# abdenlab/giql

Measured on AMD Instinct MI355X. Metric: overlap-pairs/sec, 10Mx100M INTERSECTS inner join, higher is better.
Workload: dtype int32

## Files before the change

giql_amd/csrc/giql_hip.hip:

```cpp
#include <hip/hip_runtime.h>
#include <chrono>
#include <atomic>
#include <sys/mman.h>
#include <utility>
#if defined(__SSE2__)
#include <emmintrin.h>
#endif
#include <mutex>
#include <thread>
#include <stdarg.h>
#include <stdio.h>
#include <stdlib.h>
#include <string.h>

#include <vector>

#include "../../include/giql_hip.h"
#include "aux_kernels.hip.h"
#include "take_kernels.hip.h"
#include "select_kernels.hip.h"
#include "cluster_kernels.hip.h"
#include "dev_common.hip.h"
#include "join_kernels.hip.h"
#include "onesweep.hip.h"
// ... 24 lines not shown

#define GIQL_TRY(expr)      \
  do {                      \
    int _rc = (expr);       \
    if (_rc != GIQL_OK) return _rc; \
  } while (0)

#ifndef GIQL_RC_ITEMS
#define GIQL_RC_ITEMS 1
#endif
constexpr int RC_ITEMS_C2 = GIQL_RC_ITEMS;
#ifndef GIQL_FILL_ITEMS
#define GIQL_FILL_ITEMS 16
#endif
constexpr int FILL_ITEMS_C2 = GIQL_FILL_ITEMS;

#ifndef GIQL_STREAM_GRID
#define GIQL_STREAM_GRID 16384u
#endif

static inline size_t align_up(size_t x, size_t a) { return (x + a - 1) / a * a; }
static inline u32 cdiv(u64 a, u64 b) { return (u32)((a + b - 1) / b); }

struct SortBufs {
  u32* key[2];
  u32* end[2];
  u32* rid[2];
};

struct InnerState {
  SortBufs sa, sb;
  u32 nt1 = 0, nt2 = 0;
  int c1_items = C1_ITEMS_MAX;
  u32* wlo1 = nullptr;
  u64* c1_base = nullptr;
  bool c1_fill = false;
  u32 *lo1 = nullptr, *cnt1 = nullptr;
  u64* off1 = nullptr;
  u32* wlo2 = nullptr;
  u32* lo2 = nullptr;
  u32* cnt2 = nullptr;
  u64* off2 = nullptr;
  int uniform = 0;
};

constexpr size_t C1_SMALL_ROWS = (size_t)4 << 20;
constexpr u64 OVERLAP_MAX_ROWS = (u64)4 << 20;

struct Switches {
  bool classic_sort = false;
  int os_variant = 0;
  int os_order = 2;
  u32 os_help_after = OS_HELP_AFTER;
  int inject_timeout = 0;
  bool no_uniform = false;
  bool no_span_hist = false;
  bool no_coarse_b = false;
  double coarse_max_group_rows = 8.0;
  bool no_fuse_count = false;
  bool no_local_sort = false;
  u64 local_min_rows = 1u << 21;
  double local_min_bucket_rows = 300.0;
  double local_max_bucket_rows = 2800.0;
  bool no_narrow = false;
  int force_bits = 0;
};

struct Guesses {
  bool local_sort = true;
  int os_order = 2;
  int inject_timeout = 0;
  u64 last_span = 0;
  bool last_no_irr = false;
  bool nearest_two_sorts = false;
  int nearest_aligned = -1;
  bool spec_valid = false;
  int spec_form = 0;
  i64 spec_len = 0;
  bool spec_aligned = false;
  bool spec_fuse_len_ok = false;
  bool spec_sorted[2] = {false, false};
  bool row_spec_valid = false;
  i64 row_spec_len = 0;
  int spec_misses = 0;
  int local_resorts = 0;
  int order_fallbacks = 0;
};

struct CallState {
  bool prezeroed = false;
  bool first_unstable = false;
  u32* span_hist_dirty[2] = {nullptr, nullptr};
  int force_local = 0;
  int index_bits = 16;
  bool used_sorted[2] = {false, false};
  bool last_sort_local = false;
  int last_local_bits = 16;
  bool count_fused = false;
  bool bucket_join = false;
};

struct InnerPlan {
  bool planned = false;
  bool plan_is_join = false;
  bool swapped = false;
  int32_t* fuse_a = nullptr;
// ... 331 lines not shown
    if (offs[k] > omax) omax = offs[k];
  }
  hipLaunchKernelGGL(k_chrom_offsets, dim3(1), dim3(256), 0, st, lb.gmin, lb.gmax, n_chrom, omin,
                     omax, lb.chrom_base, lb.chrom_first, ctx->d_meta, lb.len_part, nblk[0], nblk[1],
                     hist ? 1 : 0, lb.abase);
  return post_launch("spans");
}

static int run_linearize(giql_hip_ctx* ctx, hipStream_t st, const giql_side& s, int n_chrom,
                         const LinBufs& lb, u32* keys, u32* ends, u32* irr_list, int which,
                         int keep_irregular, u32* hist_partial = nullptr, u32* gbase = nullptr,
                         u32* hist_end = nullptr, u32* gbase_end = nullptr, bool skip_end = false) {
  if (s.n == 0) return GIQL_OK;
  const int* end_col = skip_end ? (const int*)nullptr : s.end;
  bool dirty = false;
  for (int k = 0; k < 2; k++)
    if (hist_partial && ctx->call.span_hist_dirty[k] == hist_partial) {
      dirty = true;
      ctx->call.span_hist_dirty[k] = nullptr;
    }
  if (hist_partial && (!ctx->call.prezeroed || dirty))
    HIP_TRY(hipMemsetAsync(hist_partial, 0, (size_t)LIN_HIST_REPLICAS * 1024 * sizeof(u32), st));
  if (hist_end && !ctx->call.prezeroed)
    HIP_TRY(hipMemsetAsync(hist_end, 0, (size_t)LIN_HIST_REPLICAS * 1024 * sizeof(u32), st));
  Phase ph(ctx, st, GIQL_PH_LINEARIZE, hist_partial ? 2 : 1);
  u32 grid = cdiv((u64)s.n, LIN_NT);
  if (grid > (u32)LIN_MAX_BLOCKS) grid = LIN_MAX_BLOCKS;
  if (hist_end)
    hipLaunchKernelGGL((k_linearize<true>), dim3(grid), dim3(LIN_NT), 0, st, s.chrom, s.start, end_col,
                       (u32)s.n, s.start_off, s.end_off, n_chrom, lb.chrom_base, keys, ends, irr_list,
                       ctx->d_meta, which, keep_irregular, hist_partial, hist_end);
  else
    hipLaunchKernelGGL((k_linearize<false>), dim3(grid), dim3(LIN_NT), 0, st, s.chrom, s.start, end_col,
                       (u32)s.n, s.start_off, s.end_off, n_chrom, lb.chrom_base, keys, ends, irr_list,
                       ctx->d_meta, which, keep_irregular, hist_partial, (u32*)nullptr);
  if (hist_partial)
    hipLaunchKernelGGL(k_digit_offsets, dim3(4), dim3(256), 0, st, hist_partial,
                       (u32)LIN_HIST_REPLICAS, gbase);
  if (hist_end)
    hipLaunchKernelGGL(k_digit_offsets, dim3(4), dim3(256), 0, st, hist_end, (u32)LIN_HIST_REPLICAS,
                       gbase_end);
  return post_launch("linearize");
}

static inline size_t os_pass_words(size_t n) {
  return (size_t)cdiv(n ? n : 1, OS_MIN_TILE) * OS_BINS + 16;
}
static inline size_t os_pass_stride(const giql_hip_ctx* ctx, size_t n) {
  return ctx->sw.os_variant == 0 ? (size_t)cdiv(n ? n : 1, 8192) * OS_BINS + 16 : os_pass_words(n);
}

template <int NT, int ITEMS>
static void launch_onesweep(giql_hip_ctx* ctx, hipStream_t st, SortBufs& sb, int src, int dst, bool first,
                            u32 n, int shift, const u32* gbase, u32* status, DevMeta* meta, int unstable = 0) {
  const u32 grid = cdiv(n, NT * ITEMS);
  u32* claim = status + os_pass_stride(ctx, n) - 16;
  const u32* rin = (first || !sb.rid[0]) ? (const u32*)nullptr : sb.rid[src];
  const int mode = (sb.rid[0] ? 1 : 0) | (sb.end[0] ? 2 : 0);
#define GIQL_OS_LAUNCH(M)                                                                            \
  hipLaunchKernelGGL((k_onesweep<M, NT, ITEMS>), dim3(grid), dim3(NT), 0, st, sb.key[src],           \
                     sb.end[0] ? sb.end[src] : (const u32*)nullptr, rin, sb.key[dst],                 \
                     sb.end[0] ? sb.end[dst] : (u32*)nullptr, sb.rid[0] ? sb.rid[dst] : (u32*)nullptr, \
                     n, shift, gbase, status, claim, meta, ctx->guess.os_order, ctx->sw.os_help_after, (const u32*)nullptr, 0u, 0u,  \
                     unstable)
  switch (mode) {
    case 0: GIQL_OS_LAUNCH(0); break;
    case 1: GIQL_OS_LAUNCH(1); break;
    case 2: GIQL_OS_LAUNCH(2); break;
    default: GIQL_OS_LAUNCH(3); break;
  }
#undef GIQL_OS_LAUNCH
}

static inline int density_bits(const giql_hip_ctx* ctx, double per_bucket) {
  int w = 16;
  while (per_bucket > ctx->sw.local_max_bucket_rows && w > BS_MIN_WBITS && !ctx->sw.no_narrow) {
    per_bucket *= 0.5;
    w--;
  }
  return per_bucket <= ctx->sw.local_max_bucket_rows ? w : 0;
}

static inline int sort_local_bits(const giql_hip_ctx* ctx, size_t n) {
  if (ctx->call.force_local > 0 && ctx->bucket_bnd && ctx->sw.os_variant == 0) return ctx->call.index_bits;
  if (ctx->call.force_local < 0) return 0;
  if (!(ctx->guess.local_sort && ctx->bucket_bnd && ctx->sw.os_variant == 0 && n >= ctx->sw.local_min_rows)) return 0;
  const double span = ctx->guess.last_span ? (double)ctx->guess.last_span : 3.2e9;
  double per_bucket = (double)n * 65536.0 / span;
  if (per_bucket < ctx->sw.local_min_bucket_rows) return 0;
  if (ctx->sw.force_bits) return ctx->sw.force_bits;
  return density_bits(ctx, per_bucket);
}
static inline int local_passes(int wbits) { return wbits == 16 ? 2 : 3; }

struct FuseCount {
  BsFuse dev;
  u32 nq_total;
  const u32* irr_q;
  const u32* gbq3;
  u32 key_mask;
  const int* len_max_q;
  u32* zero_ptr;
  u32 zero_words;
  bool join = false;
  bool general = false;
  const int* len_max_u = nullptr;
};

static int64_t bucket_stage_fused_bytes(u32 n, const FuseCount& fuse);
static void launch_bucket_stage_fused(giql_hip_ctx* ctx, hipStream_t st, SortBufs& sb, u32 n, const u32* gbase,
                                      const FuseCount& fuse_in, int wbits = 16) {
  FuseCount fuse = fuse_in;
  fuse.dev.wbits = (u32)wbits;
  const u32 BS_BUCKETS = bs_n_buckets((u32)wbits);
  ctx->stats.phase_bytes[GIQL_PH_SORT_LOCAL] += bucket_stage_fused_bytes(n, fuse);
  ctx->call.count_fused = true;
  ctx->call.bucket_join = fuse.join;
  ctx->call.last_local_bits = wbits;
  {
    Phase ph(ctx, st, GIQL_PH_COUNT, 1);
    hipLaunchKernelGGL(k_bucket_bounds_fused, dim3(cdiv((u64)3 * BS_BUCKETS + 1, 256)), dim3(256), 0, st, sb.key[0], n,
                       gbase + 3 * OS_BINS, ctx->bucket_bnd, ctx->bucket_big, fuse.dev, fuse.nq_total, fuse.irr_q,
                       fuse.gbq3, fuse.key_mask, fuse.len_max_q, fuse.zero_ptr, fuse.zero_words, fuse.len_max_u);
// ... 43 lines not shown
                             int skip_digits = 0, const FuseCount* fuse = nullptr, bool presorted = false) {
  if (n == 0) return GIQL_OK;
  if (presorted) {
    const int mode = (sb.rid[0] ? 1 : 0) | (sb.end[0] ? 2 : 0);
    const int wbits_pre = sort_local_bits(ctx, n);
    const bool local_fused = fuse && mode == (fuse->general ? 3 : 1) && wbits_pre != 0;
    {
      Phase ph(ctx, st, GIQL_PH_SORT_SCATTER, 1);
      u32 grid = cdiv(n, 256 * 8);
      if (grid > GIQL_STREAM_GRID) grid = GIQL_STREAM_GRID;
      if (keygen) {
        ctx->stats.phase_bytes[GIQL_PH_SORT_SCATTER] += (int64_t)4 * n * ((mode & 2 ? 3 : 2) + 1 + (mode & 1) + (mode & 2 ? 1 : 0));
        const u32 so = (u32)keygen->start_off, eo = (u32)keygen->end_off;
        switch (mode) {
          case 0: hipLaunchKernelGGL(k_keygen_stream<0>, dim3(grid), dim3(256), 0, st, keygen->chrom, keygen->start, keygen->end, n, abase, so, eo, sb.key[0], (u32*)nullptr, (u32*)nullptr); break;
          case 1: hipLaunchKernelGGL(k_keygen_stream<1>, dim3(grid), dim3(256), 0, st, keygen->chrom, keygen->start, keygen->end, n, abase, so, eo, sb.key[0], (u32*)nullptr, sb.rid[0]); break;
          case 2: hipLaunchKernelGGL(k_keygen_stream<2>, dim3(grid), dim3(256), 0, st, keygen->chrom, keygen->start, keygen->end, n, abase, so, eo, sb.key[0], sb.end[0], (u32*)nullptr); break;
          default: hipLaunchKernelGGL(k_keygen_stream<3>, dim3(grid), dim3(256), 0, st, keygen->chrom, keygen->start, keygen->end, n, abase, so, eo, sb.key[0], sb.end[0], sb.rid[0]); break;
        }
      } else if (sb.rid[0] && !keep_rids) {
        ctx->stats.phase_bytes[GIQL_PH_SORT_SCATTER] += (int64_t)4 * n;
        hipLaunchKernelGGL(k_iota, dim3(grid), dim3(256), 0, st, sb.rid[0], n);
      }
      GIQL_TRY(post_launch("sorted input (no sort)"));
    }
    if (!local_fused) return GIQL_OK;
    ctx->call.last_sort_local = true;
    launch_bucket_stage_fused(ctx, st, sb, n, gbase, *fuse, wbits_pre);
    return post_launch("bucket stage (sorted input, fused count)");
  }
  const int wbits = sort_local_bits(ctx, n);
  const bool local = wbits != 0;
  if (local) ctx->call.last_sort_local = true;
  if (local) skip_digits = 0;
  const int n_pass = local ? local_passes(wbits) : 4 - skip_digits;
  const int first_digit = local ? 4 - n_pass : skip_digits;
  const size_t per_pass = os_pass_stride(ctx, n);
  if (!ctx->call.prezeroed) HIP_TRY(hipMemsetAsync(status, 0, n_pass * per_pass * sizeof(u32), st));
  {
    Phase ph(ctx, st, GIQL_PH_SORT_SCATTER, n_pass);
    for (int pass = 0; pass < n_pass; pass++) {
      const int src = pass & 1, dst = src ^ 1;
      const int digit = first_digit + pass;
      u32* stat = status + pass * per_pass;
      const bool first = pass == 0 && !keep_rids;
      const u32* gb = gbase + digit * OS_BINS;
      {
        const int w_out = 1 + (sb.rid[0] ? 1 : 0) + (sb.end[0] ? 1 : 0);
        const int w_in = (pass == 0 && keygen) ? 2 + (sb.end[0] ? 1 : 0)
                                               : 1 + ((sb.rid[0] && !first) ? 1 : 0) + (sb.end[0] ? 1 : 0);
        ctx->stats.phase_bytes[GIQL_PH_SORT_SCATTER] += (int64_t)4 * (w_in + w_out) * n;
      }
      const int unstable = (pass == 0 && !keep_rids && ctx->call.first_unstable) ? 1 : 0;
      if (pass == 0 && keygen) {
        const u32 grid = cdiv(n, 1024 * 8);
        u32* claim = stat + per_pass - 16;
        if (sb.end[0])
          hipLaunchKernelGGL((k_onesweep<3, 1024, 8, true>), dim3(grid), dim3(1024), 0, st,
                             reinterpret_cast<const u32*>(keygen->start), reinterpret_cast<const u32*>(keygen->end),
                             reinterpret_cast<const u32*>(keygen->chrom), sb.key[dst], sb.end[dst], sb.rid[dst], n,
                             digit * 8, gb, stat, claim, ctx->d_meta, ctx->guess.os_order, ctx->sw.os_help_after, abase,
                             (u32)keygen->start_off, (u32)keygen->end_off, unstable);
        else
          hipLaunchKernelGGL((k_onesweep<1, 1024, 8, true>), dim3(grid), dim3(1024), 0, st,
                             reinterpret_cast<const u32*>(keygen->start), reinterpret_cast<const u32*>(keygen->chrom),
                             (const u32*)nullptr, sb.key[dst], (u32*)nullptr, sb.rid[dst], n, digit * 8, gb, stat, claim,
                             ctx->d_meta, ctx->guess.os_order, ctx->sw.os_help_after, abase, (u32)keygen->start_off, 0u, unstable);
        continue;
      }
      switch (ctx->sw.os_variant) {
        case 1: launch_onesweep<512, 8>(ctx, st, sb, src, dst, first, n, digit * 8, gb, stat, ctx->d_meta, unstable); break;
        case 2: launch_onesweep<512, 16>(ctx, st, sb, src, dst, first, n, digit * 8, gb, stat, ctx->d_meta, unstable); break;
        case 3: launch_onesweep<256, 16>(ctx, st, sb, src, dst, first, n, digit * 8, gb, stat, ctx->d_meta, unstable); break;
        case 4: launch_onesweep<1024, 4>(ctx, st, sb, src, dst, first, n, digit * 8, gb, stat, ctx->d_meta, unstable); break;
        case 5: case 7: launch_onesweep<1024, 12>(ctx, st, sb, src, dst, first, n, digit * 8, gb, stat, ctx->d_meta, unstable); break;
        default: launch_onesweep<1024, 8>(ctx, st, sb, src, dst, first, n, digit * 8, gb, stat, ctx->d_meta, unstable); break;
      }
    }
  }
  if (n_pass & 1) {
    u32* t;
    t = sb.key[0], sb.key[0] = sb.key[1], sb.key[1] = t;
    t = sb.end[0], sb.end[0] = sb.end[1], sb.end[1] = t;
    t = sb.rid[0], sb.rid[0] = sb.rid[1], sb.rid[1] = t;
  }
  if (local) {
    const int mode = (sb.rid[0] ? 1 : 0) | (sb.end[0] ? 2 : 0);
    if (fuse && mode == (fuse->general ? 3 : 1)) {
      launch_bucket_stage_fused(ctx, st, sb, n, gbase, *fuse, wbits);
      return post_launch("onesweep sort (fused count)");
    }
    BsFuse bw;
    bw.wbits = (u32)wbits;
    ctx->call.last_local_bits = wbits;
    const u32 BS_BUCKETS = bs_n_buckets((u32)wbits);
    HIP_TRY(hipMemsetAsync(ctx->bucket_big, 0, sizeof(u32), st));
    Phase ph(ctx, st, GIQL_PH_SORT_LOCAL, 3);
    ctx->stats.phase_bytes[GIQL_PH_SORT_LOCAL] +=
        (int64_t)8 * (1 + (sb.rid[0] ? 1 : 0) + (sb.end[0] ? 1 : 0)) * n;
    hipLaunchKernelGGL(k_bucket_bounds, dim3(cdiv((u64)BS_BUCKETS + 1, 256)), dim3(256), 0, st, sb.key[0], n,
                       gbase + 3 * OS_BINS, ctx->bucket_bnd, (u32)wbits);
#define GIQL_BS_LAUNCH(M)                                                                              \
  if (wbits == 16)                                                                                     \
    hipLaunchKernelGGL((k_bucket_sort<M, 0, true>), dim3(BS_BUCKETS), dim3(BS_NT), 0, st, sb.key[0],   \
                       sb.end[0] ? sb.end[0] : (u32*)nullptr, sb.rid[0] ? sb.rid[0] : (u32*)nullptr,    \
                       ctx->bucket_bnd, ctx->d_meta, ctx->bucket_big, bw);                             \
  else                                                                                                 \
  hipLaunchKernelGGL((k_bucket_sort<M>), dim3(BS_BUCKETS), dim3(BS_NT), 0, st, sb.key[0],              \
                     sb.end[0] ? sb.end[0] : (u32*)nullptr, sb.rid[0] ? sb.rid[0] : (u32*)nullptr,      \
                     ctx->bucket_bnd, ctx->d_meta, ctx->bucket_big, bw);                               \
  hipLaunchKernelGGL((k_bucket_sort_big<M>), dim3(ctx->n_cu), dim3(BS_NT), 0, st, sb.key[0],           \
                     sb.end[0] ? sb.end[0] : (u32*)nullptr, sb.rid[0] ? sb.rid[0] : (u32*)nullptr,      \
                     sb.key[1], sb.end[0] ? sb.end[1] : (u32*)nullptr, sb.rid[0] ? sb.rid[1] : (u32*)nullptr, \
                     ctx->bucket_bnd, ctx->bucket_big, bw)
    switch (mode) {
      case 0: GIQL_BS_LAUNCH(0); break;
      case 1: GIQL_BS_LAUNCH(1); break;
      case 2: GIQL_BS_LAUNCH(2); break;
      default: GIQL_BS_LAUNCH(3); break;
    }
#undef GIQL_BS_LAUNCH
  }
  return post_launch("onesweep sort");
}

static inline void adopt_by_end(SortBufs& owner, const SortBufs& by_end) {
  for (int k = 0; k < 2; k++) {
    owner.end[k] = by_end.key[k];
    owner.key[k] = by_end.end[k];
// ... 151 lines not shown
  speculated = false;
  if (ctx->sw.no_uniform) return GIQL_OK;
  if (ctx->guess.row_spec_valid) {
    uni_len = ctx->guess.row_spec_len;
    speculated = true;
    return GIQL_OK;
  }
  GIQL_TRY(read_meta(ctx, st));
  uni_len = uniform_len_b(*ctx->h_meta);
  ctx->guess.last_span = ctx->h_meta->total_span;
  return GIQL_OK;
}

static bool row_form_settled(giql_hip_ctx* ctx, i64 uni_len, bool speculated) {
  if (ctx->sw.no_uniform) return true;
  const i64 actual = uniform_len_b(*ctx->h_meta);
  const bool ok = !(speculated && uni_len != 0 && actual != uni_len);
  ctx->guess.row_spec_valid = ok;
  ctx->guess.row_spec_len = actual;
  return ok;
}

static void parse_flag(const char* v, void* f) { *(bool*)f = atoi(v) != 0; }
static void parse_int(const char* v, void* f) { *(int*)f = atoi(v); }
static void parse_u32(const char* v, void* f) { *(u32*)f = (u32)strtoul(v, nullptr, 10); }
static void parse_classic(const char* v, void* f) { *(bool*)f = strcmp(v, "classic") == 0; }
static void parse_positive(const char* v, void* f) {
  if (atof(v) > 0) *(double*)f = atof(v);
}
static void parse_nonnegative(const char* v, void* f) {
  if (atof(v) >= 0) *(double*)f = atof(v);
}
static void parse_local_bits(const char* v, void* f) {
  if (atoi(v) >= BS_MIN_WBITS && atoi(v) <= 16) *(int*)f = atoi(v);
}
static void parse_local_min_rows(const char* v, void* f) {
  Switches& s = *(Switches*)f;
  s.local_min_rows = strtoull(v, nullptr, 10);
  s.local_max_bucket_rows = 1e30;
  s.local_min_bucket_rows = 0.0;
}

static Switches read_switches() {
  Switches s;
  const struct {
    const char* name;
    void (*parse)(const char*, void*);
    void* field;
  } table[] = {
      {"GIQL_HIP_SORT", parse_classic, &s.classic_sort},
      {"GIQL_HIP_OS_VARIANT", parse_int, &s.os_variant},
      {"GIQL_HIP_OS_ORDER", parse_int, &s.os_order},
      {"GIQL_HIP_OS_HELP_AFTER", parse_u32, &s.os_help_after},
      {"GIQL_HIP_INJECT_TIMEOUT", parse_int, &s.inject_timeout},
      {"GIQL_HIP_NO_UNIFORM", parse_flag, &s.no_uniform},
      {"GIQL_HIP_NO_SPAN_HIST", parse_flag, &s.no_span_hist},
      {"GIQL_HIP_NO_COARSE_B", parse_flag, &s.no_coarse_b},
      {"GIQL_HIP_COARSE_MAX_GROUP_ROWS", parse_positive, &s.coarse_max_group_rows},
      {"GIQL_HIP_NO_FUSE_COUNT", parse_flag, &s.no_fuse_count},
      {"GIQL_HIP_NO_LOCAL_SORT", parse_flag, &s.no_local_sort},
      {"GIQL_HIP_LOCAL_MIN_ROWS", parse_local_min_rows, &s},
      {"GIQL_HIP_LOCAL_MIN_BUCKET_ROWS", parse_nonnegative, &s.local_min_bucket_rows},
      {"GIQL_HIP_LOCAL_MAX_BUCKET_ROWS", parse_positive, &s.local_max_bucket_rows},
      {"GIQL_HIP_NO_NARROW_BUCKETS", parse_flag, &s.no_narrow},
      {"GIQL_HIP_LOCAL_BITS", parse_local_bits, &s.force_bits},
  };
  for (const auto& row : table)
    if (const char* v = getenv(row.name)) row.parse(v, row.field);
  return s;
}

extern "C" {

int giql_hip_abi_version(void) { return GIQL_HIP_ABI_VERSION; }

const char* giql_hip_last_error(void) { return g_err; }

int giql_hip_device_count(int* n_devices) {
  if (!n_devices) return set_err(GIQL_ERR_INVALID, "n_devices is NULL");
  int n = 0;
  HIP_TRY(hipGetDeviceCount(&n));
  *n_devices = n;
  return GIQL_OK;
}

int giql_hip_create(int device, giql_hip_ctx** out) {
  if (!out) return set_err(GIQL_ERR_INVALID, "out is NULL");
  *out = nullptr;
  int n = 0;
  HIP_TRY(hipGetDeviceCount(&n));
  if (device < 0 || device >= n)
    return set_err(GIQL_ERR_INVALID, "device %d not in [0,%d)", device, n);
  HIP_TRY(hipSetDevice(device));
  giql_hip_ctx* ctx = new (std::nothrow) giql_hip_ctx(read_switches());
  if (!ctx) return set_err(GIQL_ERR_NOMEM, "out of host memory");
  ctx->device = device;
  memset(&ctx->stats, 0, sizeof(ctx->stats));
  {
    hipDeviceProp_t prop;
    if (hipGetDeviceProperties(&prop, device) == hipSuccess && prop.multiProcessorCount > 0)
      ctx->n_cu = prop.multiProcessorCount;
  }
  hipError_t e = hipMalloc((void**)&ctx->d_meta, sizeof(DevMeta));
  if (e == hipSuccess) e = hipHostMalloc((void**)&ctx->h_meta, sizeof(DevMeta), hipHostMallocDefault);
  if (e == hipSuccess) e = hipMalloc((void**)&ctx->d_scratch64, 64);
  if (e == hipSuccess &&
// ... 2954 lines not shown
```

giql_amd/csrc/onesweep.hip.h:

```cpp
#pragma once

#include "dev_common.hip.h"

namespace giql {

constexpr int OS_BINS = 256;
constexpr int OS_MIN_TILE = 4096;
constexpr u32 OS_FLAG_AGG = 1u << 30;
constexpr u32 OS_FLAG_PREFIX = 2u << 30;
constexpr u32 OS_VALUE_MASK = (1u << 30) - 1u;
constexpr u32 OS_MAX_ROWS = (1u << 30) - 1u;
constexpr u32 OS_NO_TILE = 0xFFFFFFFFu;
#ifndef GIQL_OS_LB_WIDTH
#define GIQL_OS_LB_WIDTH 8
#endif
constexpr int OS_LB_WIDTH = GIQL_OS_LB_WIDTH;
#ifndef GIQL_OS_PRESTAGE
#define GIQL_OS_PRESTAGE 1
#endif

constexpr u32 OS_HELP_AFTER = 1u << 11;

#if defined(GIQL_OS_TIMELINE)
constexpr u32 OS_TL_TILES = 1u << 15;
__device__ unsigned long long g_os_tl[OS_TL_TILES * 16];
#define GIQL_TL(tile, k)                                                             \
  do {                                                                               \
    if (threadIdx.x == 0 && (tile) < OS_TL_TILES) g_os_tl[(size_t)(tile) * 16 + (k)] = wall_clock64(); \
  } while (0)
#else
#define GIQL_TL(tile, k) do { } while (0)
#endif

__device__ __forceinline__ void wave_match8(u32 d, u64 active, u32& below, u32& total) {
  u32 mis_lo = 0, mis_hi = 0;
#pragma unroll
  for (int b = 0; b < 8; b++) {
    const int s = __builtin_amdgcn_sbfe((int)d, b, 1);
    const u64 m = __ballot(s != 0);
    mis_lo |= (u32)m ^ (u32)s;
    mis_hi |= (u32)(m >> 32) ^ (u32)s;
  }
  const u32 p_lo = (u32)active & ~mis_lo;
  const u32 p_hi = (u32)(active >> 32) & ~mis_hi;
  below = __builtin_amdgcn_mbcnt_hi(p_hi, __builtin_amdgcn_mbcnt_lo(p_lo, 0u));
  total = (u32)__popc(p_lo) + (u32)__popc(p_hi);
}

#ifndef GIQL_OS_XCD_GROUP
#define GIQL_OS_XCD_GROUP 16
#endif
constexpr u32 OS_GROUPS = XCD_GROUPS;
constexpr u32 OS_GROUP = GIQL_OS_XCD_GROUP;

__device__ __forceinline__ u32 os_tile_of_ticket(u32 t, u32 n_tiles) { return xcd_tile_of_block<OS_GROUP>(t, n_tiles); }

__device__ __forceinline__ void os_store(u32* p, u32 v) { *p = v; }

template <int PAYLOAD, int OS_NT, int OS_ITEMS, bool FULL, bool KEYGEN = false>
__device__ __forceinline__ u32 onesweep_tile(
    const u32* __restrict__ keys_in, const u32* __restrict__ ends_in, const u32* __restrict__ rids_in,
    u32* __restrict__ keys_out, u32* __restrict__ ends_out, u32* __restrict__ rids_out, u32 n_valid,
    u32 tile, u32 tile_base, int shift, const u32* __restrict__ gbase, u32* __restrict__ status,
    DevMeta* __restrict__ meta, u32* s_buf, u32 (*s_wcnt)[OS_BINS], u32* s_dstart, u32* s_goff,
    u32* s_scan, u32* s_help, u32 help_after, u32 n_total, const u32* s_abase = nullptr, u32 start_off = 0,
    u32 end_off = 0, const bool unstable = false) {
  constexpr int OS_NW = OS_NT / WAVE;
  const u32 tid = threadIdx.x;
  const u32 lane = lane_id();
  const u32 w = wave_id();

  u32 key[OS_ITEMS];
  const u32 wbase = w * (OS_ITEMS * WAVE);
  const u32* kin = keys_in + tile_base;
  const u32* ein = (PAYLOAD & 2) ? ends_in + tile_base : nullptr;
  const u32* rin = ((PAYLOAD & 1) && rids_in && !KEYGEN) ? rids_in + tile_base : nullptr;
  const int* cin = KEYGEN ? reinterpret_cast<const int*>((PAYLOAD & 2) ? rids_in : ends_in) + tile_base : nullptr;
  if (KEYGEN) {
    u32 cc[OS_ITEMS];
#pragma unroll
    for (int i = 0; i < OS_ITEMS; i++) {
      const u32 r = wbase + i * WAVE + lane;
      const bool ok = FULL || r < n_valid;
      cc[i] = ok ? (u32)cin[r] : 0u;
      key[i] = ok ? kin[r] : 0u;
    }
    __syncthreads();
#pragma unroll
    for (int i = 0; i < OS_ITEMS; i++) {
      const u32 r = wbase + i * WAVE + lane;
      const bool ok = FULL || r < n_valid;
      key[i] = ok ? s_abase[cc[i] & 31u] + key[i] + start_off : U32_MAX;
    }
  } else {
#pragma unroll
    for (int i = 0; i < OS_ITEMS; i++) {
      const u32 r = wbase + i * WAVE + lane;
      const bool ok = FULL || r < n_valid;
      key[i] = ok ? kin[r] : U32_MAX;
    }
    __syncthreads();
  }

  GIQL_TL(tile, 1);
#if defined(GIQL_OS_TIMELINE)
  __builtin_amdgcn_s_waitcnt(0);
  GIQL_TL(tile, 2);
#endif
  u32 rank[OS_ITEMS];
  if (unstable) {
    u32* wcnt = s_wcnt[w];
#pragma unroll
    for (int i = 0; i < OS_ITEMS; i++) {
      const u32 r = wbase + i * WAVE + lane;
      const bool ok = FULL || r < n_valid;
      rank[i] = ok ? atomicAdd(&wcnt[(key[i] >> shift) & 0xFFu], 1u) : 0u;
    }
  } else {
    u32* wcnt = s_wcnt[w];
#pragma unroll
    for (int i = 0; i < OS_ITEMS; i++) {
      const u32 r = wbase + i * WAVE + lane;
      const bool ok = FULL || r < n_valid;
      const u32 d = (key[i] >> shift) & 0xFFu;
      const u64 active = FULL ? ~0ull : __ballot(ok);
      u32 below, total;
#if defined(GIQL_ABLATE) && GIQL_ABLATE == 2
      below = lane;
      total = 64;
      (void)active;
#else
      wave_match8(d, active, below, total);
#endif
      rank[i] = 0;
      if (ok) {
        const u32 pre = wcnt[d];
        rank[i] = pre + below;
        if (below == 0) wcnt[d] = pre + total;
      }
    }
  }
  GIQL_TL(tile, 3);
  __syncthreads();
  GIQL_TL(tile, 4);

  u32 lb_count = 0;
#if defined(GIQL_OS_FAKE_SEG)
  u32 lb_fake = 0;
#endif
  if (tid < OS_BINS) {
    u32 run = 0;
#pragma unroll
    for (int k = 0; k < OS_NW; k++) {
      const u32 c = s_wcnt[k][tid];
      s_wcnt[k][tid] = run;
      run += c;
    }
    const u32 count = run;
    lb_count = count;
    GIQL_TL(tile, 5);
    const u32 incl = wave_incl_scan(count);
    if (lane == WAVE - 1) s_scan[w] = incl;
#if !(defined(GIQL_ABLATE) && GIQL_ABLATE == 1)
#if defined(GIQL_OS_FAKE_SEG)
    {
      const u32 n_tiles_ = (n_total + (u32)(OS_NT * OS_ITEMS) - 1u) / (u32)(OS_NT * OS_ITEMS);
      const u32 bin_ = (tid == OS_BINS - 1 ? n_total : gbase[tid + 1]) - gbase[tid];
      const u32 fake_ = (u32)((u64)bin_ * tile / n_tiles_);
      const bool head_ = (tile % GIQL_OS_FAKE_SEG) == 0;
      lb_fake = head_ ? fake_ : 0u;
      __hip_atomic_store(status + (size_t)tile * OS_BINS + tid,
                         (head_ ? OS_FLAG_PREFIX : OS_FLAG_AGG) | ((count + lb_fake) & OS_VALUE_MASK), __ATOMIC_RELAXED,
                         __HIP_MEMORY_SCOPE_AGENT);
    }
#else
    __hip_atomic_store(status + (size_t)tile * OS_BINS + tid, (tile == 0 ? OS_FLAG_PREFIX : OS_FLAG_AGG) | count,
                       __ATOMIC_RELAXED, __HIP_MEMORY_SCOPE_AGENT);
#endif
#endif
    s_dstart[tid] = incl - count;
  }
  __syncthreads();
  if (tid < OS_BINS) {
    u32 wb = 0;
#pragma unroll
    for (int k = 0; k < OS_BINS / WAVE; k++)
      if (k < (int)w) wb += s_scan[k];
    s_dstart[tid] += wb;
  }
  __syncthreads();
  GIQL_TL(tile, 6);

  u32 pos[OS_ITEMS];
#pragma unroll
  for (int i = 0; i < OS_ITEMS; i++) {
    const u32 d = (key[i] >> shift) & 0xFFu;
    pos[i] = s_dstart[d] + s_wcnt[w][d] + rank[i];
  }
  u32 pay[OS_ITEMS];
  if (PAYLOAD & 2) {
#pragma unroll
    for (int i = 0; i < OS_ITEMS; i++) {
      const u32 r = wbase + i * WAVE + lane;
      if (KEYGEN)
        pay[i] = (FULL || r < n_valid) ? s_abase[(u32)cin[r] & 31u] + ein[r] + end_off : 0u;
      else
        pay[i] = (FULL || r < n_valid) ? ein[r] : 0u;
    }
  } else if (PAYLOAD & 1) {
#pragma unroll
    for (int i = 0; i < OS_ITEMS; i++) {
      const u32 r = wbase + i * WAVE + lane;
      pay[i] = (FULL || r < n_valid) ? (rin ? rin[r] : tile_base + r) : 0u;
    }
  }
#pragma unroll
  for (int i = 0; i < OS_ITEMS; i++) {
    const u32 r = wbase + i * WAVE + lane;
    if (FULL || r < n_valid) s_buf[pos[i]] = key[i];
  }
  GIQL_TL(tile, 7);
  constexpr bool PRESTAGE = GIQL_OS_PRESTAGE && (PAYLOAD == 1 || PAYLOAD == 2);
  u32 ks[PRESTAGE ? OS_ITEMS : 1], ps[PRESTAGE ? OS_ITEMS : 1];
  if (PRESTAGE) {
    __syncthreads();
#pragma unroll
    for (int i = 0; i < OS_ITEMS; i++) {
      const u32 p = i * OS_NT + tid;
      ks[i] = (FULL || p < n_valid) ? s_buf[p] : 0u;
    }
    __syncthreads();
#pragma unroll
    for (int i = 0; i < OS_ITEMS; i++) {
      const u32 r = wbase + i * WAVE + lane;
      if (FULL || r < n_valid) s_buf[pos[i]] = pay[i];
    }
    __syncthreads();
#pragma unroll
    for (int i = 0; i < OS_ITEMS; i++) {
      const u32 p = i * OS_NT + tid;
      ps[i] = (FULL || p < n_valid) ? s_buf[p] : 0u;
    }
  }
  GIQL_TL(tile, 8);
  if (tid < OS_BINS) {
    u32 excl = 0;
#if defined(GIQL_OS_FAKE_SEG)
    excl = lb_fake;
#endif
#if defined(GIQL_ABLATE) && GIQL_ABLATE == 1
    excl = tile * 32;
#else
#if defined(GIQL_OS_FAKE_SEG)
    if ((tile % GIQL_OS_FAKE_SEG) != 0) {
#else
    if (tile != 0) {
#endif
      u32* st = status + (size_t)tile * OS_BINS + tid;
      const u32 count = lb_count;
      u32 t = tile;
      u32 spins = 0;
      bool done = false;
#if defined(GIQL_OS_TIMELINE)
      u32 tl_polls = 0;
#endif
      while (!done) {
#if defined(GIQL_OS_TIMELINE)
        tl_polls++;
#endif
        u32 v[OS_LB_WIDTH];
#pragma unroll
        for (int j = 0; j < OS_LB_WIDTH; j++) {
          const u32 tj = t > (u32)j ? t - 1 - j : 0u;
          v[j] = __hip_atomic_load(status + (size_t)tj * OS_BINS + tid, __ATOMIC_RELAXED,
                                   __HIP_MEMORY_SCOPE_AGENT);
        }
        int used = 0;
#pragma unroll
        for (int j = 0; j < OS_LB_WIDTH; j++) {
          if (done || used != j) continue;
          if (t <= (u32)j) {
            done = true;
            continue;
          }
          const u32 f = v[j] >> 30;
          if (f == 0) continue;
          excl += v[j] & OS_VALUE_MASK;
          used = j + 1;
          if (f == 2u) done = true;
        }
        t -= (u32)used;
        if (!done && used == 0) {
          if (++spins > help_after) {
            atomicMin(s_help, t - 1u);
            break;
          }
          __builtin_amdgcn_s_sleep(1);
        }
        if (t == 0) done = true;
      }
      if (done)
        __hip_atomic_store(st, OS_FLAG_PREFIX | ((excl + count) & OS_VALUE_MASK), __ATOMIC_RELAXED,
                           __HIP_MEMORY_SCOPE_AGENT);
#if defined(GIQL_OS_TIMELINE)
      if (tid == 0 && tile < OS_TL_TILES) {
        g_os_tl[(size_t)tile * 16 + 12] = tl_polls;
        g_os_tl[(size_t)tile * 16 + 13] = tile - t;
      }
#endif
    }
#endif
    s_goff[tid] = gbase[tid] + excl - s_dstart[tid];
  }
  GIQL_TL(tile, 9);
  __syncthreads();
  {
    const u32 help = *s_help;
    if (help != OS_NO_TILE) return help;
  }
#if defined(GIQL_ABLATE) && GIQL_ABLATE == 3
  if (key[0] != 0x12345u) return OS_NO_TILE;
#endif
  if (PRESTAGE) {
    u32* pout = (PAYLOAD & 2) ? ends_out : rids_out;
#pragma unroll
    for (int i = 0; i < OS_ITEMS; i++) {
      const u32 p = i * OS_NT + tid;
      if (FULL || p < n_valid) {
        const u32 d = s_goff[(ks[i] >> shift) & 0xFFu] + p;
        os_store(keys_out + d, ks[i]);
        os_store(pout + d, ps[i]);
      }
    }
    GIQL_TL(tile, 10);
#if defined(GIQL_OS_TIMELINE)
    __builtin_amdgcn_s_waitcnt(0);
    GIQL_TL(tile, 11);
#endif
    return OS_NO_TILE;
  }
  u32 dst[OS_ITEMS];
#pragma unroll
  for (int i = 0; i < OS_ITEMS; i++) {
    const u32 p = i * OS_NT + tid;
    dst[i] = 0;
    if (FULL || p < n_valid) {
      const u32 k = s_buf[p];
      dst[i] = s_goff[(k >> shift) & 0xFFu] + p;
      os_store(keys_out + dst[i], k);
    }
  }
  GIQL_TL(tile, 9);
  if (PAYLOAD == 3) {
    u32 pay2[OS_ITEMS];
#pragma unroll
    for (int i = 0; i < OS_ITEMS; i++) {
      const u32 r = wbase + i * WAVE + lane;
      pay2[i] = (FULL || r < n_valid) ? (rin ? rin[r] : tile_base + r) : 0u;
    }
    __syncthreads();
#pragma unroll
    for (int i = 0; i < OS_ITEMS; i++) {
      const u32 r = wbase + i * WAVE + lane;
      if (FULL || r < n_valid) s_buf[pos[i]] = pay[i];
    }
    __syncthreads();
#pragma unroll
    for (int i = 0; i < OS_ITEMS; i++) {
      const u32 p = i * OS_NT + tid;
      if (FULL || p < n_valid) os_store(ends_out + dst[i], s_buf[p]);
    }
    __syncthreads();
#pragma unroll
    for (int i = 0; i < OS_ITEMS; i++) {
      const u32 r = wbase + i * WAVE + lane;
      if (FULL || r < n_valid) s_buf[pos[i]] = pay2[i];
    }
    __syncthreads();
#pragma unroll
    for (int i = 0; i < OS_ITEMS; i++) {
      const u32 p = i * OS_NT + tid;
      if (FULL || p < n_valid) os_store(rids_out + dst[i], s_buf[p]);
    }
  } else if (PAYLOAD != 0) {
    u32* out = (PAYLOAD & 2) ? ends_out : rids_out;
    __syncthreads();
#pragma unroll
    for (int i = 0; i < OS_ITEMS; i++) {
      const u32 r = wbase + i * WAVE + lane;
      if (FULL || r < n_valid) s_buf[pos[i]] = pay[i];
    }
    __syncthreads();
#pragma unroll
    for (int i = 0; i < OS_ITEMS; i++) {
      const u32 p = i * OS_NT + tid;
      if (FULL || p < n_valid) os_store(out + dst[i], s_buf[p]);
    }
  }
  GIQL_TL(tile, 10);
#if defined(GIQL_OS_TIMELINE)
  __builtin_amdgcn_s_waitcnt(0);
  GIQL_TL(tile, 11);
#endif
  return OS_NO_TILE;
}

template <int PAYLOAD, int OS_NT, int OS_ITEMS, bool KEYGEN = false>
__device__ __forceinline__ u32 os_run_tile(
    const u32* __restrict__ keys_in, const u32* __restrict__ ends_in, const u32* __restrict__ rids_in,
    u32* __restrict__ keys_out, u32* __restrict__ ends_out, u32* __restrict__ rids_out, u32 n, u32 tile,
    int shift, const u32* __restrict__ gbase, u32* __restrict__ status, DevMeta* __restrict__ meta,
    u32* s_buf, u32 (*s_wcnt)[OS_BINS], u32* s_dstart, u32* s_goff, u32* s_scan, u32* s_help,
    u32 help_after, const u32* s_abase = nullptr, u32 start_off = 0, u32 end_off = 0, const bool unstable = false) {
  constexpr int OS_TILE = OS_NT * OS_ITEMS;
  const u32 tile_base = tile * OS_TILE;
  const u32 n_valid = (n - tile_base) < (u32)OS_TILE ? (n - tile_base) : (u32)OS_TILE;
  if (n_valid == (u32)OS_TILE)
    return onesweep_tile<PAYLOAD, OS_NT, OS_ITEMS, true, KEYGEN>(keys_in, ends_in, rids_in, keys_out, ends_out,
                                                                 rids_out, n_valid, tile, tile_base, shift, gbase,
                                                                 status, meta, s_buf, s_wcnt, s_dstart, s_goff,
                                                                 s_scan, s_help, help_after, n, s_abase, start_off, end_off,
                                                                 unstable);
  return onesweep_tile<PAYLOAD, OS_NT, OS_ITEMS, false, KEYGEN>(keys_in, ends_in, rids_in, keys_out, ends_out,
                                                                rids_out, n_valid, tile, tile_base, shift, gbase,
                                                                status, meta, s_buf, s_wcnt, s_dstart, s_goff,
                                                                s_scan, s_help, help_after, n, s_abase, start_off, end_off,
                                                                unstable);
}

template <int PAYLOAD, int OS_NT, int OS_ITEMS, bool KEYGEN = false>
__device__ __noinline__ void os_help_loop(
    const u32* __restrict__ keys_in, const u32* __restrict__ ends_in, const u32* __restrict__ rids_in,
    u32* __restrict__ keys_out, u32* __restrict__ ends_out, u32* __restrict__ rids_out, u32 n, u32 own,
    u32 need, int shift, const u32* __restrict__ gbase, u32* __restrict__ status,
    DevMeta* __restrict__ meta, u32* s_buf, u32 (*s_wcnt)[OS_BINS], u32* s_dstart, u32* s_goff,
    u32* s_scan, u32* s_help, u32 help_after, const u32* s_abase = nullptr, u32 start_off = 0, u32 end_off = 0,
    const bool unstable = false) {
  constexpr int OS_NW = OS_NT / WAVE;
  const u32 tid = threadIdx.x;
  u32 cur = need;
  for (u32 rounds = 0;; rounds++) {
    __syncthreads();
#pragma unroll
    for (int k = tid; k < OS_NW * OS_BINS; k += OS_NT) (&s_wcnt[0][0])[k] = 0;
    if (tid == 0) *s_help = OS_NO_TILE;
    __syncthreads();
    const u32 r = os_run_tile<PAYLOAD, OS_NT, OS_ITEMS, KEYGEN>(keys_in, ends_in, rids_in, keys_out, ends_out,
                                                               rids_out, n, cur, shift, gbase, status, meta, s_buf,
                                                               s_wcnt, s_dstart, s_goff, s_scan, s_help, help_after,
                                                               s_abase, start_off, end_off, unstable);
    if (r == OS_NO_TILE) {
      if (cur == own) return;
      cur = own;
    } else {
      cur = r;
      if (rounds > (1u << 20)) {
        if (tid == 0) meta->status = -2;
        return;
      }
    }
  }
}

template <int PAYLOAD, int OS_NT, int OS_ITEMS, bool KEYGEN = false>
__global__ __launch_bounds__(OS_NT, (OS_NT == 1024 && (PAYLOAD != 3 || OS_ITEMS <= 8)) ? 8 : 1) void k_onesweep(
    const u32* __restrict__ keys_in, const u32* __restrict__ ends_in, const u32* __restrict__ rids_in,
    u32* __restrict__ keys_out, u32* __restrict__ ends_out, u32* __restrict__ rids_out, u32 n,
    int shift, const u32* __restrict__ gbase, u32* __restrict__ status, u32* __restrict__ ticket,
    DevMeta* __restrict__ meta, int order, u32 help_after, const u32* __restrict__ abase = nullptr,
    u32 start_off = 0, u32 end_off = 0, int unstable = 0) {
  constexpr int OS_TILE = OS_NT * OS_ITEMS;
  constexpr int OS_NW = OS_NT / WAVE;
  __shared__ u32 s_buf[OS_TILE];
  __shared__ u32 s_wcnt[OS_NW][OS_BINS];
  __shared__ u32 s_dstart[OS_BINS];
  __shared__ u32 s_goff[OS_BINS];
  __shared__ u32 s_scan[OS_BINS / WAVE + 1];
  __shared__ u32 s_tile;
  __shared__ u32 s_help;
  __shared__ u32 s_abase[KEYGEN ? 32 : 1];

  const u32 tid = threadIdx.x;
  if (KEYGEN && tid < 32) s_abase[tid] = abase[tid];
  if (tid == 0) {
    if (order != 2) s_tile = atomicAdd(ticket, 1u);
    s_help = OS_NO_TILE;
  }
#pragma unroll
  for (int k = tid; k < OS_NW * OS_BINS; k += OS_NT) (&s_wcnt[0][0])[k] = 0;
  if (order != 2) __syncthreads();
  const u32 own = order == 2 ? xcd_tile_of_block<OS_GROUP>(blockIdx.x, gridDim.x) : s_tile;
  if (own * OS_TILE >= n) return;
  GIQL_TL(own, 0);
  const u32 need = os_run_tile<PAYLOAD, OS_NT, OS_ITEMS, KEYGEN>(keys_in, ends_in, rids_in, keys_out, ends_out,
                                                                rids_out, n, own, shift, gbase, status, meta, s_buf,
                                                                s_wcnt, s_dstart, s_goff, s_scan, &s_help, help_after,
                                                                s_abase, start_off, end_off, unstable != 0);
  if (need != OS_NO_TILE)
    os_help_loop<PAYLOAD, OS_NT, OS_ITEMS, KEYGEN>(keys_in, ends_in, rids_in, keys_out, ends_out, rids_out, n, own,
                                                   need, shift, gbase, status, meta, s_buf, s_wcnt, s_dstart,
                                                   s_goff, s_scan, &s_help, help_after, s_abase, start_off, end_off,
                                                   unstable != 0);
}

template <int PAYLOAD>
__global__ __launch_bounds__(256) void k_keygen_stream(const int* __restrict__ chrom, const int* __restrict__ start,
                                                        const int* __restrict__ end, u32 n,
                                                        const u32* __restrict__ abase, u32 start_off, u32 end_off,
                                                        u32* __restrict__ keys, u32* __restrict__ ends,
                                                        u32* __restrict__ rids) {
  __shared__ u32 s_abase[32];
  if (threadIdx.x < 32) s_abase[threadIdx.x] = abase[threadIdx.x];
  __syncthreads();
  const u32 stride = gridDim.x * 256u;
  for (u32 i = blockIdx.x * 256u + threadIdx.x; i < n; i += stride) {
    const u32 b = s_abase[(u32)chrom[i] & 31u];
    keys[i] = b + (u32)start[i] + start_off;
    if (PAYLOAD & 2) ends[i] = b + (u32)end[i] + end_off;
    if (PAYLOAD & 1) rids[i] = i;
  }
}

__global__ __launch_bounds__(256) void k_iota(u32* __restrict__ out, u32 n) {
  const u32 stride = gridDim.x * 256u;
  for (u32 i = blockIdx.x * 256u + threadIdx.x; i < n; i += stride) out[i] = i;
}

}
```

Baseline: 198.5 billion.

## Use unchained atomic-cursor scatter for unstable first onesweep pass

For the unstable first radix pass, tiles no longer use the decoupled look-back prefix chain. Each tile instead claims its output range per bin with a relaxed atomic fetch-add on a strided global cursor. This removes serial waiting on predecessor tiles and the help loop. The cost is nondeterministic ordering within a bin (acceptable because the pass is already unstable) and atomic contention on the per-bin cursors. The path is gated by an env flag, the default variant and a minimum tile count.

```diff
diff --git a/giql_amd/csrc/giql_hip.hip b/giql_amd/csrc/giql_hip.hip
--- a/giql_amd/csrc/giql_hip.hip
+++ b/giql_amd/csrc/giql_hip.hip
@@ -100,6 +100,7 @@
   int os_variant = 0;
   int os_order = 2;
   u32 os_help_after = OS_HELP_AFTER;
+  bool chained_first_pass = false;
   int inject_timeout = 0;
   bool no_uniform = false;
   bool no_span_hist = false;
@@ -537,23 +538,33 @@
 
 template <int NT, int ITEMS>
 static void launch_onesweep(giql_hip_ctx* ctx, hipStream_t st, SortBufs& sb, int src, int dst, bool first,
-                            u32 n, int shift, const u32* gbase, u32* status, DevMeta* meta, int unstable = 0) {
+                            u32 n, int shift, const u32* gbase, u32* status, DevMeta* meta, int unstable = 0,
+                            bool unchained = false) {
   const u32 grid = cdiv(n, NT * ITEMS);
   u32* claim = status + os_pass_stride(ctx, n) - 16;
   const u32* rin = (first || !sb.rid[0]) ? (const u32*)nullptr : sb.rid[src];
   const int mode = (sb.rid[0] ? 1 : 0) | (sb.end[0] ? 2 : 0);
 #define GIQL_OS_LAUNCH(M)                                                                            \
-  hipLaunchKernelGGL((k_onesweep<M, NT, ITEMS>), dim3(grid), dim3(NT), 0, st, sb.key[src],           \
+  hipLaunchKernelGGL((k_onesweep<M, NT, ITEMS, false, UNCHAINED>), dim3(grid), dim3(NT), 0, st, sb.key[src], \
                      sb.end[0] ? sb.end[src] : (const u32*)nullptr, rin, sb.key[dst],                 \
                      sb.end[0] ? sb.end[dst] : (u32*)nullptr, sb.rid[0] ? sb.rid[dst] : (u32*)nullptr, \
                      n, shift, gbase, status, claim, meta, ctx->guess.os_order, ctx->sw.os_help_after, (const u32*)nullptr, 0u, 0u,  \
                      unstable)
-  switch (mode) {
-    case 0: GIQL_OS_LAUNCH(0); break;
-    case 1: GIQL_OS_LAUNCH(1); break;
-    case 2: GIQL_OS_LAUNCH(2); break;
-    default: GIQL_OS_LAUNCH(3); break;
-  }
+#define GIQL_OS_LAUNCH_MODE()         \
+  switch (mode) {                     \
+    case 0: GIQL_OS_LAUNCH(0); break; \
+    case 1: GIQL_OS_LAUNCH(1); break; \
+    case 2: GIQL_OS_LAUNCH(2); break; \
+    default: GIQL_OS_LAUNCH(3); break; \
+  }
+  if (NT == 1024 && ITEMS == 8 && unchained) {
+    constexpr bool UNCHAINED = NT == 1024 && ITEMS == 8;
+    GIQL_OS_LAUNCH_MODE()
+  } else {
+    constexpr bool UNCHAINED = false;
+    GIQL_OS_LAUNCH_MODE()
+  }
+#undef GIQL_OS_LAUNCH_MODE
 #undef GIQL_OS_LAUNCH
 }
 
@@ -703,20 +714,29 @@
         ctx->stats.phase_bytes[GIQL_PH_SORT_SCATTER] += (int64_t)4 * (w_in + w_out) * n;
       }
       const int unstable = (pass == 0 && !keep_rids && ctx->call.first_unstable) ? 1 : 0;
+      const bool unchained = unstable && !ctx->sw.chained_first_pass && ctx->sw.os_variant == 0 &&
+                             cdiv(n, 1024 * 8) >= OS_UNCHAINED_MIN_TILES;
       if (pass == 0 && keygen) {
         const u32 grid = cdiv(n, 1024 * 8);
         u32* claim = stat + per_pass - 16;
-        if (sb.end[0])
-          hipLaunchKernelGGL((k_onesweep<3, 1024, 8, true>), dim3(grid), dim3(1024), 0, st,
-                             reinterpret_cast<const u32*>(keygen->start), reinterpret_cast<const u32*>(keygen->end),
-                             reinterpret_cast<const u32*>(keygen->chrom), sb.key[dst], sb.end[dst], sb.rid[dst], n,
-                             digit * 8, gb, stat, claim, ctx->d_meta, ctx->guess.os_order, ctx->sw.os_help_after, abase,
-                             (u32)keygen->start_off, (u32)keygen->end_off, unstable);
-        else
-          hipLaunchKernelGGL((k_onesweep<1, 1024, 8, true>), dim3(grid), dim3(1024), 0, st,
-                             reinterpret_cast<const u32*>(keygen->start), reinterpret_cast<const u32*>(keygen->chrom),
-                             (const u32*)nullptr, sb.key[dst], (u32*)nullptr, sb.rid[dst], n, digit * 8, gb, stat, claim,
-                             ctx->d_meta, ctx->guess.os_order, ctx->sw.os_help_after, abase, (u32)keygen->start_off, 0u, unstable);
+#define GIQL_OS_KEYGEN_LAUNCH(U)                                                                                        \
+  if (sb.end[0])                                                                                                        \
+    hipLaunchKernelGGL((k_onesweep<3, 1024, 8, true, U>), dim3(grid), dim3(1024), 0, st,                                \
+                       reinterpret_cast<const u32*>(keygen->start), reinterpret_cast<const u32*>(keygen->end),          \
+                       reinterpret_cast<const u32*>(keygen->chrom), sb.key[dst], sb.end[dst], sb.rid[dst], n,           \
+                       digit * 8, gb, stat, claim, ctx->d_meta, ctx->guess.os_order, ctx->sw.os_help_after, abase,      \
+                       (u32)keygen->start_off, (u32)keygen->end_off, unstable);                                         \
+  else                                                                                                                  \
+    hipLaunchKernelGGL((k_onesweep<1, 1024, 8, true, U>), dim3(grid), dim3(1024), 0, st,                                \
+                       reinterpret_cast<const u32*>(keygen->start), reinterpret_cast<const u32*>(keygen->chrom),        \
+                       (const u32*)nullptr, sb.key[dst], (u32*)nullptr, sb.rid[dst], n, digit * 8, gb, stat, claim,     \
+                       ctx->d_meta, ctx->guess.os_order, ctx->sw.os_help_after, abase, (u32)keygen->start_off, 0u, unstable)
+        if (unchained) {
+          GIQL_OS_KEYGEN_LAUNCH(true);
+        } else {
+          GIQL_OS_KEYGEN_LAUNCH(false);
+        }
+#undef GIQL_OS_KEYGEN_LAUNCH
         continue;
       }
       switch (ctx->sw.os_variant) {
@@ -725,7 +745,7 @@
         case 3: launch_onesweep<256, 16>(ctx, st, sb, src, dst, first, n, digit * 8, gb, stat, ctx->d_meta, unstable); break;
         case 4: launch_onesweep<1024, 4>(ctx, st, sb, src, dst, first, n, digit * 8, gb, stat, ctx->d_meta, unstable); break;
         case 5: case 7: launch_onesweep<1024, 12>(ctx, st, sb, src, dst, first, n, digit * 8, gb, stat, ctx->d_meta, unstable); break;
-        default: launch_onesweep<1024, 8>(ctx, st, sb, src, dst, first, n, digit * 8, gb, stat, ctx->d_meta, unstable); break;
+        default: launch_onesweep<1024, 8>(ctx, st, sb, src, dst, first, n, digit * 8, gb, stat, ctx->d_meta, unstable, unchained); break;
       }
     }
   }
@@ -983,6 +1003,7 @@
       {"GIQL_HIP_OS_VARIANT", parse_int, &s.os_variant},
       {"GIQL_HIP_OS_ORDER", parse_int, &s.os_order},
       {"GIQL_HIP_OS_HELP_AFTER", parse_u32, &s.os_help_after},
+      {"GIQL_HIP_CHAINED_FIRST_PASS", parse_flag, &s.chained_first_pass},
       {"GIQL_HIP_INJECT_TIMEOUT", parse_int, &s.inject_timeout},
       {"GIQL_HIP_NO_UNIFORM", parse_flag, &s.no_uniform},
       {"GIQL_HIP_NO_SPAN_HIST", parse_flag, &s.no_span_hist},
diff --git a/giql_amd/csrc/onesweep.hip.h b/giql_amd/csrc/onesweep.hip.h
--- a/giql_amd/csrc/onesweep.hip.h
+++ b/giql_amd/csrc/onesweep.hip.h
@@ -19,16 +19,20 @@
 #define GIQL_OS_PRESTAGE 1
 #endif
 
+constexpr u32 OS_CURSOR_STRIDE = 32;
+constexpr u32 OS_UNCHAINED_MIN_TILES = OS_CURSOR_STRIDE;
 constexpr u32 OS_HELP_AFTER = 1u << 11;
 
 #if defined(GIQL_OS_TIMELINE)
 constexpr u32 OS_TL_TILES = 1u << 15;
 __device__ unsigned long long g_os_tl[OS_TL_TILES * 16];
+#define GIQL_TL_PASS(unstable_pass) const bool tl_on = (GIQL_OS_TIMELINE + 0) != 2 || (unstable_pass)
 #define GIQL_TL(tile, k)                                                             \
   do {                                                                               \
-    if (threadIdx.x == 0 && (tile) < OS_TL_TILES) g_os_tl[(size_t)(tile) * 16 + (k)] = wall_clock64(); \
+    if (threadIdx.x == 0 && tl_on && (tile) < OS_TL_TILES) g_os_tl[(size_t)(tile) * 16 + (k)] = wall_clock64(); \
   } while (0)
 #else
+#define GIQL_TL_PASS(unstable_pass) do { } while (0)
 #define GIQL_TL(tile, k) do { } while (0)
 #endif
 
@@ -57,7 +61,7 @@
 
 __device__ __forceinline__ void os_store(u32* p, u32 v) { *p = v; }
 
-template <int PAYLOAD, int OS_NT, int OS_ITEMS, bool FULL, bool KEYGEN = false>
+template <int PAYLOAD, int OS_NT, int OS_ITEMS, bool FULL, bool KEYGEN = false, bool UNCHAINED = false>
 __device__ __forceinline__ u32 onesweep_tile(
     const u32* __restrict__ keys_in, const u32* __restrict__ ends_in, const u32* __restrict__ rids_in,
     u32* __restrict__ keys_out, u32* __restrict__ ends_out, u32* __restrict__ rids_out, u32 n_valid,
@@ -69,6 +73,7 @@
   const u32 tid = threadIdx.x;
   const u32 lane = lane_id();
   const u32 w = wave_id();
+  GIQL_TL_PASS(UNCHAINED || unstable);
 
   u32 key[OS_ITEMS];
   const u32 wbase = w * (OS_ITEMS * WAVE);
@@ -108,7 +113,7 @@
   GIQL_TL(tile, 2);
 #endif
   u32 rank[OS_ITEMS];
-  if (unstable) {
+  if (UNCHAINED || unstable) {
     u32* wcnt = s_wcnt[w];
 #pragma unroll
     for (int i = 0; i < OS_ITEMS; i++) {
@@ -161,6 +166,11 @@
     GIQL_TL(tile, 5);
     const u32 incl = wave_incl_scan(count);
     if (lane == WAVE - 1) s_scan[w] = incl;
+    if (UNCHAINED) {
+      lb_count = count ? __hip_atomic_fetch_add(status + tid * OS_CURSOR_STRIDE, count, __ATOMIC_RELAXED,
+                                                __HIP_MEMORY_SCOPE_AGENT)
+                       : 0u;
+    } else {
 #if !(defined(GIQL_ABLATE) && GIQL_ABLATE == 1)
 #if defined(GIQL_OS_FAKE_SEG)
     {
@@ -178,6 +188,7 @@
                        __ATOMIC_RELAXED, __HIP_MEMORY_SCOPE_AGENT);
 #endif
 #endif
+    }
     s_dstart[tid] = incl - count;
   }
   __syncthreads();
@@ -243,7 +254,12 @@
     }
   }
   GIQL_TL(tile, 8);
-  if (tid < OS_BINS) {
+  if (UNCHAINED) {
+    if (tid < OS_BINS) s_goff[tid] = gbase[tid] + lb_count - s_dstart[tid];
+#if defined(GIQL_OS_TIMELINE)
+    if (tid == 0 && tl_on && tile < OS_TL_TILES) g_os_tl[(size_t)tile * 16 + 12] = g_os_tl[(size_t)tile * 16 + 13] = 0;
+#endif
+  } else if (tid < OS_BINS) {
     u32 excl = 0;
 #if defined(GIQL_OS_FAKE_SEG)
     excl = lb_fake;
@@ -303,7 +319,7 @@
         __hip_atomic_store(st, OS_FLAG_PREFIX | ((excl + count) & OS_VALUE_MASK), __ATOMIC_RELAXED,
                            __HIP_MEMORY_SCOPE_AGENT);
 #if defined(GIQL_OS_TIMELINE)
-      if (tid == 0 && tile < OS_TL_TILES) {
+      if (tid == 0 && tl_on && tile < OS_TL_TILES) {
         g_os_tl[(size_t)tile * 16 + 12] = tl_polls;
         g_os_tl[(size_t)tile * 16 + 13] = tile - t;
       }
@@ -314,7 +330,7 @@
   }
   GIQL_TL(tile, 9);
   __syncthreads();
-  {
+  if (!UNCHAINED) {
     const u32 help = *s_help;
     if (help != OS_NO_TILE) return help;
   }
@@ -405,7 +421,7 @@
   return OS_NO_TILE;
 }
 
-template <int PAYLOAD, int OS_NT, int OS_ITEMS, bool KEYGEN = false>
+template <int PAYLOAD, int OS_NT, int OS_ITEMS, bool KEYGEN = false, bool UNCHAINED = false>
 __device__ __forceinline__ u32 os_run_tile(
     const u32* __restrict__ keys_in, const u32* __restrict__ ends_in, const u32* __restrict__ rids_in,
     u32* __restrict__ keys_out, u32* __restrict__ ends_out, u32* __restrict__ rids_out, u32 n, u32 tile,
@@ -416,16 +432,12 @@
   const u32 tile_base = tile * OS_TILE;
   const u32 n_valid = (n - tile_base) < (u32)OS_TILE ? (n - tile_base) : (u32)OS_TILE;
   if (n_valid == (u32)OS_TILE)
-    return onesweep_tile<PAYLOAD, OS_NT, OS_ITEMS, true, KEYGEN>(keys_in, ends_in, rids_in, keys_out, ends_out,
-                                                                 rids_out, n_valid, tile, tile_base, shift, gbase,
-                                                                 status, meta, s_buf, s_wcnt, s_dstart, s_goff,
-                                                                 s_scan, s_help, help_after, n, s_abase, start_off, end_off,
-                                                                 unstable);
-  return onesweep_tile<PAYLOAD, OS_NT, OS_ITEMS, false, KEYGEN>(keys_in, ends_in, rids_in, keys_out, ends_out,
-                                                                rids_out, n_valid, tile, tile_base, shift, gbase,
-                                                                status, meta, s_buf, s_wcnt, s_dstart, s_goff,
-                                                                s_scan, s_help, help_after, n, s_abase, start_off, end_off,
-                                                                unstable);
+    return onesweep_tile<PAYLOAD, OS_NT, OS_ITEMS, true, KEYGEN, UNCHAINED>(
+        keys_in, ends_in, rids_in, keys_out, ends_out, rids_out, n_valid, tile, tile_base, shift, gbase, status, meta,
+        s_buf, s_wcnt, s_dstart, s_goff, s_scan, s_help, help_after, n, s_abase, start_off, end_off, unstable);
+  return onesweep_tile<PAYLOAD, OS_NT, OS_ITEMS, false, KEYGEN, UNCHAINED>(
+      keys_in, ends_in, rids_in, keys_out, ends_out, rids_out, n_valid, tile, tile_base, shift, gbase, status, meta,
+      s_buf, s_wcnt, s_dstart, s_goff, s_scan, s_help, help_after, n, s_abase, start_off, end_off, unstable);
 }
 
 template <int PAYLOAD, int OS_NT, int OS_ITEMS, bool KEYGEN = false>
@@ -462,7 +474,7 @@
   }
 }
 
-template <int PAYLOAD, int OS_NT, int OS_ITEMS, bool KEYGEN = false>
+template <int PAYLOAD, int OS_NT, int OS_ITEMS, bool KEYGEN = false, bool UNCHAINED = false>
 __global__ __launch_bounds__(OS_NT, (OS_NT == 1024 && (PAYLOAD != 3 || OS_ITEMS <= 8)) ? 8 : 1) void k_onesweep(
     const u32* __restrict__ keys_in, const u32* __restrict__ ends_in, const u32* __restrict__ rids_in,
     u32* __restrict__ keys_out, u32* __restrict__ ends_out, u32* __restrict__ rids_out, u32 n,
@@ -491,12 +503,12 @@
   if (order != 2) __syncthreads();
   const u32 own = order == 2 ? xcd_tile_of_block<OS_GROUP>(blockIdx.x, gridDim.x) : s_tile;
   if (own * OS_TILE >= n) return;
+  GIQL_TL_PASS(UNCHAINED || unstable != 0);
   GIQL_TL(own, 0);
-  const u32 need = os_run_tile<PAYLOAD, OS_NT, OS_ITEMS, KEYGEN>(keys_in, ends_in, rids_in, keys_out, ends_out,
-                                                                rids_out, n, own, shift, gbase, status, meta, s_buf,
-                                                                s_wcnt, s_dstart, s_goff, s_scan, &s_help, help_after,
-                                                                s_abase, start_off, end_off, unstable != 0);
-  if (need != OS_NO_TILE)
+  const u32 need = os_run_tile<PAYLOAD, OS_NT, OS_ITEMS, KEYGEN, UNCHAINED>(
+      keys_in, ends_in, rids_in, keys_out, ends_out, rids_out, n, own, shift, gbase, status, meta, s_buf, s_wcnt,
+      s_dstart, s_goff, s_scan, &s_help, help_after, s_abase, start_off, end_off, unstable != 0);
+  if (!UNCHAINED && need != OS_NO_TILE)
     os_help_loop<PAYLOAD, OS_NT, OS_ITEMS, KEYGEN>(keys_in, ends_in, rids_in, keys_out, ends_out, rids_out, n, own,
                                                    need, shift, gbase, status, meta, s_buf, s_wcnt, s_dstart,
                                                    s_goff, s_scan, &s_help, help_after, s_abase, start_off, end_off,
```

Result: slower. 184.2 billion (-7.2%).
